# VitorMPCastro/MessyerRaytracer

Measured on AMD Instinct MI355X. Metric: Mrays/s (primary, closest-hit), higher is better.
Workload: dtype f32

## Files before the change

__graft_entry__.py:

```python
import os
import sys

ROOT = os.path.dirname(os.path.abspath(__file__))
if ROOT not in sys.path:
    sys.path.insert(0, ROOT)


def build() -> None:
    from messyerraytracer_amd import build as b
    b.build_lib()
    b.build_host_test()
    b.build_host_cpu_test()
    b.build_host_tlas_test()
    b.build_policy_test()
    b.build_shadow_policy_test()
    b.build_reflection_policy_test()
    b.build_hemisphere_policy_test()
    b.build_bounce_policy_test()
    b.build_instance_math_test()
    b.build_shade_data_test()
    from oracle import pyoracle
    pyoracle.build(force=False)
    if os.path.isdir("/root/reference") and not pyoracle.ref_available():
        pyoracle.build(force=True)
    import messyerraytracer_amd
    from messyerraytracer_amd import capi
    L = capi.load()
    missing = [s for s in capi.SYMBOLS if not hasattr(L, s)]
    if missing:
        raise RuntimeError(f"libmrt_hip.so does not export {missing}")


def smoke() -> None:
    import numpy as np
    from messyerraytracer_amd import capi, synth
    from oracle import pyoracle as po

    ctx = capi.Context(0)
    for verts, (w, h), origin, fwd, fov in (
            (synth.cube(), (16, 12), (0, 0, 3), (0, 0, -1), 60.0),
            (synth.soup(2000, 0.4, 3), (128, 96), (0, 0, -12), (0, 0, 1), 50.0)):
        scene = capi.Scene(verts)
        scene.upload(ctx)
        cam = capi.camera_look(origin, fwd, w, h, fov)
        got = ctx.cast_grid(cam, w, h)
        osc = po.OracleScene(verts)
        rays = po.grid_rays(origin, fwd, w, h, fov)
        want = osc.trace(rays)
        assert (got["prim_id"] == want["prim_id"]).all(), "prim_id mismatch vs oracle"
        hit = want["prim_id"] >= 0
        assert np.array_equal(got["t"][hit], want["t"][hit]), "t mismatch vs oracle"
        assert hit.any() and (~hit).any()
    local, inst = synth.multi_mesh_instances(4, 500, 0.3, 5)
# ... 30 lines not shown
```

messyerraytracer_amd/build.py:

```python
import concurrent.futures
import os
import shutil
import subprocess

HERE = os.path.dirname(os.path.abspath(__file__))
CSRC = os.path.join(HERE, "csrc")
LIB = os.path.join(HERE, "libmrt_hip.so")
OBJ = os.path.join(HERE, "_obj")
HOST_TEST = os.path.join(HERE, "host_mirror_test")
HOST_CPU_TEST = os.path.join(HERE, "host_cpu_test")
HOST_TLAS_TEST = os.path.join(HERE, "host_tlas_test")
POLICY_TEST = os.path.join(HERE, "launch_policy_test")
SHADOW_POLICY_TEST = os.path.join(HERE, "shadow_policy_test")
REFLECTION_POLICY_TEST = os.path.join(HERE, "reflection_policy_test")
HEMISPHERE_POLICY_TEST = os.path.join(HERE, "hemisphere_policy_test")
BOUNCE_POLICY_TEST = os.path.join(HERE, "bounce_policy_test")
INSTANCE_MATH_TEST = os.path.join(HERE, "instance_math_test")
SHADE_DATA_TEST = os.path.join(HERE, "shade_data_test")

SOURCES = ["kernels.hip", "api.hip", "cast.hip", "schedule.hip", "launch_policy.cpp", "group.hip", "device_build.hip", "refit.hip",
           "tlas_device.hip", "surface.hip", "host/shade_data.cpp", "host/scene_prep.cpp", "host/bvh_builder.cpp", "host/two_level_prep.cpp"]
HEADERS = ["mrt_internal.h", "instance_math.h", "mrt_context.h", "launch_policy.h", "packet_kernel.h", "packet_asm_kernel.h", "packet_rows_kernel.h", "packet_quad_kernel.h", "two_level_kernel.h", "lane_persistent_kernel.h", "source_common.h", "shadow_kernel.h", "reflection_kernel.h", "hemisphere_kernel.h", "bounce_kernel.h", "surface_kernel.h", "shade_data.h", "lane_walk.inc", "two_level_walk.inc", "persistent_walk.inc", "../../include/mrt_hip.h", "host/gpu_ray_caster.hpp", "host/ray_dispatcher.hpp",
           "host/host_types.hpp", "host/cpu_backend.hpp", "host/ray_tracer_server.hpp", "host/record_policy_test.h"]
FLAGS = ["--offload-arch=gfx950", "-O3", "-std=c++17", "-fPIC", "-ffp-contract=off", "-Wall",
         "-Wno-unused-result", "-Xarch_host", "-mfma"]


def _hipcc() -> str:
    for c in (shutil.which("hipcc"), "/opt/rocm/bin/hipcc"):
        if c and os.path.exists(c):
            return c
    raise RuntimeError("hipcc not found: libmrt_hip.so cannot be built")


def _stale(target: str, deps) -> bool:
    if not os.path.exists(target):
        return True
    t = os.path.getmtime(target)
    return any(os.path.exists(d) and os.path.getmtime(d) > t for d in deps)


def build_lib(force: bool = False, verbose: bool = False) -> str:
    srcs = [os.path.join(CSRC, s) for s in SOURCES]
    deps = srcs + [os.path.join(CSRC, h) for h in HEADERS] + [os.path.abspath(__file__)]
    if force or _stale(LIB, deps):
        extra = ["-DMRT_WITH_QUAD"] if os.environ.get("MRT_WITH_QUAD") == "1" else []
        extra += os.environ.get("MRT_EXTRA_DEFINES", "").split()
        os.makedirs(OBJ, exist_ok=True)
        objs = [os.path.join(OBJ, s.replace("/", "_") + ".o") for s in SOURCES]

        def compile_one(job):
            src, obj = job
            cmd = [_hipcc()] + FLAGS + extra + ["-c", src, "-o", obj]
            r = subprocess.run(cmd, capture_output=True, text=True, cwd=CSRC)
            if r.returncode != 0:
# ... 92 lines not shown


def build_bounce_policy_test(force: bool = False) -> str:
    srcs = [os.path.join(CSRC, "host", "bounce_policy_test.cpp"), os.path.join(CSRC, "launch_policy.cpp")]
    deps = srcs + [os.path.join(CSRC, h) for h in HEADERS]
    if force or _stale(BOUNCE_POLICY_TEST, deps):
        cmd = [_hipcc(), "-O2", "-std=c++17", "-Wall"] + srcs + ["-o", BOUNCE_POLICY_TEST]
        r = subprocess.run(cmd, capture_output=True, text=True, cwd=CSRC)
        if r.returncode != 0:
            raise RuntimeError("bounce policy test build failed:\n" + r.stdout + r.stderr)
    return BOUNCE_POLICY_TEST


def build_instance_math_test(force: bool = False) -> str:
    src = os.path.join(CSRC, "host", "instance_math_test.cpp")
    deps = [src, os.path.join(CSRC, "instance_math.h")]
    if force or _stale(INSTANCE_MATH_TEST, deps):
        cmd = [_hipcc(), "-x", "c++", "-O2", "-std=c++17", "-ffp-contract=off", "-Wall", src, "-o", INSTANCE_MATH_TEST]
        r = subprocess.run(cmd, capture_output=True, text=True, cwd=CSRC)
        if r.returncode != 0:
            raise RuntimeError("instance math test build failed:\n" + r.stdout + r.stderr)
    return INSTANCE_MATH_TEST


def build_shade_data_test(force: bool = False) -> str:
    srcs = [os.path.join(CSRC, "host", "shade_data_test.cpp"), os.path.join(CSRC, "host", "shade_data.cpp")]
    deps = srcs + [os.path.join(CSRC, "shade_data.h"), os.path.join(CSRC, "../../include/mrt_hip.h")]
    if force or _stale(SHADE_DATA_TEST, deps):
        cmd = [_hipcc(), "-x", "c++", "-O2", "-std=c++17", "-ffp-contract=off", "-Wall"] + srcs + ["-o", SHADE_DATA_TEST]
        r = subprocess.run(cmd, capture_output=True, text=True, cwd=CSRC)
        if r.returncode != 0:
            raise RuntimeError("shade data test build failed:\n" + r.stdout + r.stderr)
    return SHADE_DATA_TEST


if __name__ == "__main__":
    print(build_lib(force=True, verbose=True))
    print(build_host_test(force=True))
    print(build_host_cpu_test(force=True))
    print(build_host_tlas_test(force=True))
    print(build_policy_test(force=True))
    print(build_shadow_policy_test(force=True))
    print(build_reflection_policy_test(force=True))
    print(build_hemisphere_policy_test(force=True))
    print(build_bounce_policy_test(force=True))
    print(build_instance_math_test(force=True))
    print(build_shade_data_test(force=True))
```

messyerraytracer_amd/csrc/kernels.hip:

```cpp
#include <hip/hip_runtime.h>
#include <cfloat>
#include <cstdarg>
#include <cstdio>
#include <cstdlib>
#include <type_traits>
#include "mrt_internal.h"
#include "shade_data.h"

namespace mrt {

#define MRT_WG 256
#define MRT_WAVE 64

__device__ __forceinline__ float fma_(float a, float b, float c) { return __builtin_fmaf(a, b, c); }
__device__ __forceinline__ float dot3(float ax, float ay, float az, float bx, float by, float bz)
{
	return fma_(ax, bx, fma_(ay, by, az * bz));
}
__device__ __forceinline__ float safe_inv(float d)
{
	const float eps = 1e-9f;
	const float big = 1.0f / eps;
	return __builtin_fabsf(d) > eps ? 1.0f / d : (d >= 0.0f ? big : -big);
}

struct RayRegs {
	float ox, oy, oz, dx, dy, dz, t_min, t_max;
};

__device__ __forceinline__ bool skip_launch(const TraceParams &p)
{
	return p.skip_flag != nullptr && *p.skip_flag == p.skip_when;
}

__device__ __forceinline__ bool lane_ray_index_g(const TraceParams &p, uint64_t g, uint64_t &ray_idx, uint32_t &px, uint32_t &py);
__device__ __forceinline__ bool lane_ray_index(const TraceParams &p, uint32_t block, uint64_t &ray_idx, uint32_t &px, uint32_t &py)
{
	return lane_ray_index_g(p, (uint64_t)block * MRT_WG + threadIdx.x, ray_idx, px, py);
}
__device__ __forceinline__ bool xcd_strips(const TraceParams &p, uint64_t tile, uint32_t tiles_x, uint32_t tiles_y, uint32_t &tx, uint32_t &ty)
{
	const uint32_t tg = p.tile_group ? p.tile_group : 1u;
	uint32_t m = (tiles_x + 128u) >> 8;
	if (m == 0u) m = 1u;
	const uint32_t S = tiles_x / (8u * m);
	if (S == 0u || S * 8u * m != tiles_x || S % tg != 0u) return false;
	const uint64_t wg = tile / tg;
	const uint32_t k = (uint32_t)wg & 7u;
	const uint64_t j = (wg >> 3) * tg + tile % tg;
	const uint64_t per_strip = (uint64_t)S * tiles_y;
	const uint32_t sl = (uint32_t)(j / per_strip), r = (uint32_t)(j % per_strip);
	ty = r / S;
	tx = (sl * 8u + k) * S + r % S;
	return true;
}

__device__ __forceinline__ bool lane_ray_index_g(const TraceParams &p, uint64_t g, uint64_t &ray_idx, uint32_t &px, uint32_t &py)
{
	uint32_t lane_map = p.lane_map, grid_w = p.grid_w, rows = p.rows, tiles_x = p.tiles_x;
	if (lane_map == MAP_AUTO) {
		const uint32_t w = p.auto_grid[0];
		lane_map = w ? MAP_TILE8X8 : MAP_LINEAR;
		grid_w = w; rows = p.auto_grid[1]; tiles_x = p.auto_grid[2];
	}
	if (lane_map == MAP_TILE8X8) {
		uint64_t tile = g >> 6;
		const uint32_t l = (uint32_t)g & 63u;
		uint32_t tx, ty;
		const uint32_t k = p.tile_w_log2;
		const uint32_t tiles_y = (rows + (64u >> k) - 1u) >> (6u - k);
		uint32_t quarter = 4u;
		uint32_t sixteenth = 16u;
		if (p.quarter_all == 2u) { sixteenth = (uint32_t)tile & 15u; tile >>= 4; if (l >= 4u || tile >= (uint64_t)tiles_x * tiles_y) return false; }
		else if (p.quarter_all) { quarter = (uint32_t)tile & 3u; tile >>= 2; if (l >= 16u || tile >= (uint64_t)tiles_x * tiles_y) return false; }
		else if (p.tile_sched != nullptr && ((uint64_t)tiles_x * tiles_y + p.tile_unit - 1u) / p.tile_unit == p.n_units) {
			const uint64_t slot = tile / p.tile_unit;
			if (slot >= (p.sched_hdr ? p.sched_hdr[2] : p.n_units)) return false;
			const uint32_t e = p.tile_sched[slot], what = e >> 28, id = e & 0x0FFFFFFFu;
			if (what == 0u) tile = (uint64_t)id * p.tile_unit + tile % p.tile_unit;
			else {
				if (tile % p.tile_unit != 0u) return false;
				tile = id;
				if (what >= 2u) { quarter = what - 2u; if (l >= 16u) return false; }
			}
		}
		if (p.tile_order == 1u && (tiles_x & 15u) == 0u && (tiles_y & 15u) == 0u) {
			const uint32_t st = (uint32_t)(tile >> 8), in = (uint32_t)tile & 255u;
			uint32_t mx = in & 0x55u, my = (in >> 1) & 0x55u;
			mx = (mx | (mx >> 1)) & 0x33u; mx = (mx | (mx >> 2)) & 0x0Fu;
			my = (my | (my >> 1)) & 0x33u; my = (my | (my >> 2)) & 0x0Fu;
			const uint32_t stx = st % (tiles_x >> 4), sty = st / (tiles_x >> 4);
			tx = (stx << 4) + mx; ty = (sty << 4) + my;
		} else if (p.tile_order == 2u && (tiles_x & 31u) == 0u && (tiles_y & 31u) == 0u) {
			const uint32_t st = (uint32_t)(tile >> 10), in = (uint32_t)tile & 1023u;
			uint32_t mx = in & 0x155u, my = (in >> 1) & 0x155u;
			mx = (mx | (mx >> 1)) & 0x133u; mx = (mx | (mx >> 2)) & 0x10Fu; mx = (mx | (mx >> 4)) & 0x1Fu;
			my = (my | (my >> 1)) & 0x133u; my = (my | (my >> 2)) & 0x10Fu; my = (my | (my >> 4)) & 0x1Fu;
			const uint32_t stx = st % (tiles_x >> 5), sty = st / (tiles_x >> 5);
			tx = (stx << 5) + mx; ty = (sty << 5) + my;
		} else if (p.tile_order == 3u && xcd_strips(p, tile, tiles_x, tiles_y, tx, ty)) {
		} else { tx = (uint32_t)(tile % tiles_x); ty = (uint32_t)(tile / tiles_x); }
		if (sixteenth < 16u) {
			px = (tx << 3) + ((sixteenth & 3u) << 1) + (l & 1u);
			py = (ty << 3) + ((sixteenth >> 2) << 1) + (l >> 1);
		} else if (quarter < 4u) {
			px = (tx << 3) + ((quarter & 1u) << 2) + (l & 3u);
			py = (ty << 3) + ((quarter >> 1) << 2) + (l >> 2);
		} else {
			px = (tx << k) + (l & ((1u << k) - 1u));
			py = (ty << (6u - k)) + (l >> k);
		}
		if (px >= grid_w || py >= rows) return false;
		ray_idx = (uint64_t)py * grid_w + px;
		return true;
	}
	if (p.sparse_lanes) { const uint32_t l = (uint32_t)g & 63u; if (l >= p.sparse_lanes) return false; g = (g >> 6) * p.sparse_lanes + l; }
	if (g >= p.count) return false;
	ray_idx = p.perm ? (uint64_t)p.perm[g] : g;
	if (p.in_fmt == IN_GRID) { px = (uint32_t)(ray_idx % p.grid_w); py = (uint32_t)(ray_idx / p.grid_w); }
	return true;
}

__device__ __forceinline__ bool tile_cost_word(const TraceParams &p, uint64_t g_first, uint32_t *&park, uint32_t *&sum, uint32_t &what)
{
	if (p.tile_cost == nullptr) return false;
	uint32_t rows = p.rows, tiles_x = p.tiles_x;
	if (p.lane_map == MAP_AUTO) { if (p.auto_grid[0] == 0u) return false; rows = p.auto_grid[1]; tiles_x = p.auto_grid[2]; }
	else if (p.lane_map != MAP_TILE8X8) return false;
	const uint32_t k = p.tile_w_log2, tiles_y = (rows + (64u >> k) - 1u) >> (6u - k);
	if (((uint64_t)tiles_x * tiles_y + p.tile_unit - 1u) / p.tile_unit != p.n_units) return false;
	const uint64_t slot = (g_first >> 6) / p.tile_unit;
	what = 0u;
	if (p.tile_sched == nullptr) { if (slot >= p.n_units) return false; park = sum = p.tile_cost + slot; return true; }
	if (slot >= (p.sched_hdr ? p.sched_hdr[2] : p.n_units)) return false;
	const uint32_t e = p.tile_sched[slot], id = e & 0x0FFFFFFFu;
	what = e >> 28;
	if (what == 0u) { park = sum = p.tile_cost + id; return true; }
	park = p.tile_cost + p.n_units + slot;
	sum = p.tile_cost + id / p.tile_unit;
	return true;
}
__device__ __forceinline__ void note_tile_start(const TraceParams &p, uint64_t g_first)
{
	uint32_t *park, *sum, what;
	if (tile_cost_word(p, g_first, park, sum, what)) *park = (uint32_t)__builtin_amdgcn_s_memtime();
}
__device__ __forceinline__ void note_tile_cost(const TraceParams &p, uint64_t g_first)
{
	uint32_t *park, *sum, what;
	if (!tile_cost_word(p, g_first, park, sum, what)) return;
	uint32_t d = (uint32_t)__builtin_amdgcn_s_memtime() - *park;
	if (park == sum) { *sum = d ? d : 1u; return; }
	if (what == 1u) d = d - (d >> 2);
	else d = p.tile_unit == 2u ? (d >> 1) + (d >> 3) + (d >> 4) : d - (d >> 3);
	atomicAdd(sum, d ? d : 1u);
}

__device__ __forceinline__ void grid_ray(const TraceParams &p, uint32_t px, uint32_t py, RayRegs &r)
{
	const mrt_camera &c = p.cam;
	float dx, dy, dz;
	r.ox = c.origin[0]; r.oy = c.origin[1]; r.oz = c.origin[2];
	if (c.kind == MRT_CAMERA_DEBUG_GRID) {
		const float u = (2.0f * ((float)px + 0.5f) / (float)p.grid_w - 1.0f) * c.half_w;
		const float v = (2.0f * ((float)(py + p.y0) + 0.5f) / (float)p.grid_h - 1.0f) * c.half_h;
		dx = c.fwd[0] + c.right[0] * u + c.up[0] * v;
		dy = c.fwd[1] + c.right[1] * u + c.up[1] * v;
		dz = c.fwd[2] + c.right[2] * u + c.up[2] * v;
	} else {
		const float u = (2.0f * ((float)px + c.jitter_x) * c.inv_w) - 1.0f;
		const float v = 1.0f - (2.0f * ((float)(py + p.y0) + c.jitter_y) * c.inv_h);
		if (c.kind == MRT_CAMERA_PERSPECTIVE) {
			const float vx = u * c.half_w, vy = v * c.half_h;
			dx = c.right[0] * vx + c.up[0] * vy + c.fwd[0] * -1.0f;
			dy = c.right[1] * vx + c.up[1] * vy + c.fwd[1] * -1.0f;
			dz = c.right[2] * vx + c.up[2] * vy + c.fwd[2] * -1.0f;
		} else {
			const float sv = v * c.half_h, su = u * c.half_w;
			r.ox = (c.origin[0] + c.up[0] * sv) + c.right[0] * su;
			r.oy = (c.origin[1] + c.up[1] * sv) + c.right[1] * su;
			r.oz = (c.origin[2] + c.up[2] * sv) + c.right[2] * su;
			r.dx = -c.fwd[0]; r.dy = -c.fwd[1]; r.dz = -c.fwd[2];
			r.t_min = c.t_min; r.t_max = c.t_max;
			return;
		}
	}
	const float l2 = dx * dx + dy * dy + dz * dz;
	if (l2 == 0.0f) { dx = dy = dz = 0.0f; }
	else { const float l = __builtin_sqrtf(l2); dx /= l; dy /= l; dz /= l; }
	r.dx = dx; r.dy = dy; r.dz = dz;
	r.t_min = c.t_min; r.t_max = c.t_max;
}

__device__ __forceinline__ void load_ray(const TraceParams &p, uint64_t idx, uint32_t px, uint32_t py, RayRegs &r)
{
	if (p.in_fmt == IN_GRID) { grid_ray(p, px, py, r); return; }
	float ox, oy, oz, dx, dy, dz, t0, t1;
	if (p.in_fmt == IN_HOST60) {
		const float *h = reinterpret_cast<const float *>(p.rays) + idx * 15u;
		ox = h[0]; oy = h[1]; oz = h[2]; dx = h[3]; dy = h[4]; dz = h[5];
		t0 = h[12]; t1 = h[13];
	} else {
		const float4 *q = reinterpret_cast<const float4 *>(p.rays) + idx * 2u;
		const float4 a = q[0], b = q[1];
		ox = a.x; oy = a.y; oz = a.z; t1 = a.w;
		dx = b.x; dy = b.y; dz = b.z; t0 = b.w;
	}
	r.ox = ox; r.oy = oy; r.oz = oz; r.dx = dx; r.dy = dy; r.dz = dz; r.t_min = t0; r.t_max = t1;
}

__device__ __forceinline__ void store_hit(const TraceParams &p, uint64_t idx, const RayRegs &r,
		float t, int32_t prim, float u, float v, float nx, float ny, float nz, uint32_t layers, uint32_t slot)
{
	if (p.out_fmt == OUT_BOOL8) { reinterpret_cast<uint8_t *>(p.hits)[idx] = prim >= 0 ? 1 : 0; return; }
	if (p.out_fmt == OUT_TOKEN4) { reinterpret_cast<uint32_t *>(p.hits)[idx] = prim >= 0 ? slot : 0xFFFFFFFFu; return; }
	if (p.out_fmt == OUT_HOST44) {
		float *h = reinterpret_cast<float *>(p.hits) + idx * 11u;
		uint32_t *hu = reinterpret_cast<uint32_t *>(h);
		if (prim >= 0) {
			h[0] = t;
			h[1] = r.ox + r.dx * t; h[2] = r.oy + r.dy * t; h[3] = r.oz + r.dz * t;
			h[4] = nx; h[5] = ny; h[6] = nz; h[7] = u; h[8] = v;
			hu[9] = (uint32_t)prim; hu[10] = layers;
		} else {
			h[0] = FLT_MAX; h[1] = h[2] = h[3] = 0.0f; h[4] = h[5] = h[6] = 0.0f; h[7] = h[8] = 0.0f;
			hu[9] = 0xFFFFFFFFu; hu[10] = 0u;
		}
		return;
	}
	float4 *q = reinterpret_cast<float4 *>(p.hits) + idx * 2u;
	float4 a, b;
	a.x = t; a.y = __int_as_float(prim); a.z = u; a.w = v;
	b.x = nx; b.y = ny; b.z = nz; b.w = __uint_as_float(layers);
	q[0] = a; q[1] = b;
}

__device__ __forceinline__ void finish_ray(const TraceParams &p, uint64_t ray_idx, const RayRegs &r,
		float best_t, float best_u, float best_v, uint32_t best_slot)
{
	int32_t prim = -1; float nx = 0.0f, ny = 0.0f, nz = 0.0f; uint32_t layers = 0u;
	if (best_slot != 0xFFFFFFFFu) {
		if (p.out_fmt == OUT_BOOL8 || p.out_fmt == OUT_TOKEN4) prim = 0;
		else {
			prim = (int32_t)p.tri_hot[best_slot].id;
			layers = p.tri_hot[best_slot].layers;
			const float4 nn = reinterpret_cast<const float4 *>(p.tri_cold)[best_slot];
			nx = nn.x; ny = nn.y; nz = nn.z;
		}
	}
	store_hit(p, ray_idx, r, best_t, prim, best_u, best_v, nx, ny, nz, layers, best_slot);
}

__device__ __forceinline__ void finish_two_level_ray(const TraceParams &p, uint64_t ray_idx, const RayRegs &r,
		float best_t, float best_u, float best_v, uint32_t best_slot, uint32_t best_id, uint32_t best_inst)
{
	int32_t prim = -1; float nx = 0.0f, ny = 0.0f, nz = 0.0f; uint32_t layers = 0u;
	if (p.out_fmt == OUT_TOKEN8) {
		reinterpret_cast<uint2 *>(p.hits)[ray_idx] = make_uint2(best_slot, best_slot != 0xFFFFFFFFu ? best_inst : 0u);
		return;
	}
	if (best_slot != 0xFFFFFFFFu) {
		prim = (int32_t)best_id;
		if (p.out_fmt != OUT_BOOL8) {
			const float4 *row = reinterpret_cast<const float4 *>(p.instances) + (size_t)best_inst * 8u;
			const float4 b0 = row[3], b1 = row[4], b2 = row[5];
			const float4 no = reinterpret_cast<const float4 *>(p.tri_cold)[best_slot];
			nx = fma_(b0.x, no.x, fma_(b0.y, no.y, b0.z * no.z));
// ... 631 lines not shown
```

messyerraytracer_amd/csrc/packet_rows_kernel.h:

```cpp
#pragma once

#define RA_LMINX "s20"
#define RA_LMINY "s21"
#define RA_LMINZ "s22"
#define RA_LREF "s23"
#define RA_LMAXX "s24"
#define RA_LMAXY "s25"
#define RA_LMAXZ "s26"
#define RA_RREF "s27"
#define RA_RMINX "s28"
#define RA_RMINY "s29"
#define RA_RMINZ "s30"
#define RA_RMAXX "s32"
#define RA_RMAXY "s33"
#define RA_RMAXZ "s34"
#define RA_MASK "s[60:61]"
#define RA_MASKLO "s60"
#define RA_MASKHI "s61"
#define RA_V0X "s20"
#define RA_V0Y "s21"
#define RA_V0Z "s22"
#define RA_ID "s23"
#define RA_E1X "s24"
#define RA_E1Y "s25"
// ... 646 lines not shown
	if (__ballot(!inside) != 0ull || !planes_ok) return c;
	const float n1 = __builtin_fabsf(n[0]) + __builtin_fabsf(n[1]) + __builtin_fabsf(n[2]);
	const float o1 = __builtin_fabsf(ox) + __builtin_fabsf(oy) + __builtin_fabsf(oz);
	const float err = 8.0f * 5.9604645e-8f * n1 * (scene_abs_max + o1);
	const float cc = (n[0] * ox + n[1] * oy + n[2] * oz) - err;
	if (__ballot(!__builtin_isfinite(cc)) != 0ull) return c;
	const uint32_t d = lane & 15u, axis = d & 3u;
	const bool is_max = (d >> 2 & 1u) != 0u;
	const float na = axis == 0u ? n[0] : (axis == 1u ? n[1] : n[2]);
	c.w = (axis < 3u && ((na >= 0.0f) == is_max)) ? na : 0.0f;
	c.cc = (d == 7u || d == 15u) ? cc : -__builtin_inff();
	return c;
}

__device__ __forceinline__ void rows_init(PacketRegs &s, const RayRegs &r, bool takes_part, uint32_t sp)
{
	s.ox = r.ox; s.oy = r.oy; s.oz = r.oz; s.dx = r.dx; s.dy = r.dy; s.dz = r.dz; s.tmin = r.t_min;
	s.ix = safe_inv(r.dx); s.iy = safe_inv(r.dy); s.iz = safe_inv(r.dz);
	s.nrx = -(r.ox * s.ix); s.nry = -(r.oy * s.iy); s.nrz = -(r.oz * s.iz);
	s.bt = r.t_max; s.bu = 0.0f; s.bv = 0.0f; s.bs = 0xFFFFFFFFu; s.bi = 0xFFFFFFFFu;
	s.lim = (!takes_part || r.t_min >= r.t_max) ? -FLT_MAX : r.t_max;
	s.sp = sp; s.cur = 0u; s.mask = 0ull;
}

__device__ __forceinline__ int rows_octant(const RayRegs &r, bool part, unsigned long long &part_mask)
{
	part_mask = __ballot(part);
	const unsigned long long sx = __ballot(part && safe_inv(r.dx) < 0.0f), sy = __ballot(part && safe_inv(r.dy) < 0.0f),
			sz = __ballot(part && safe_inv(r.dz) < 0.0f);
	const bool uniform = (sx == 0ull || sx == part_mask) && (sy == 0ull || sy == part_mask) && (sz == 0ull || sz == part_mask);
	return uniform ? ((sx ? 1 : 0) | (sy ? 2 : 0) | (sz ? 4 : 0)) : 8;
}

#ifndef MRT_ROWS_WPE
#define MRT_ROWS_WPE 8
#endif
template <bool ANY_HIT, bool COUNT, int PACKETS, int WG, bool CULL = false>
__global__ __launch_bounds__(WG) __attribute__((amdgpu_waves_per_eu(MRT_ROWS_WPE, 8))) void trace_packet_rows_kernel(const TraceParams p)
{
	__shared__ __attribute__((aligned(16))) uint32_t wave_stack[WG / MRT_WAVE][PACKETS][(MRT_PACKET_STACK + 1) * 4];
	if (skip_launch(p)) return;
	uint32_t block = blockIdx.x;
	if (p.xcd_swizzle) {
		const uint32_t per = gridDim.x >> 3;
		if (block < (per << 3)) block = (block & 7u) * per + (block >> 3);
	}
	const uint32_t wave = threadIdx.x / MRT_WAVE, lane = threadIdx.x & (MRT_WAVE - 1);
	const uint32_t wave_s = __builtin_amdgcn_readfirstlane(wave), block_s = block;
	const uint64_t g_a = (((uint64_t)block * (WG / MRT_WAVE) + wave) * PACKETS) * MRT_WAVE + lane, g_b = g_a + MRT_WAVE;
	uint64_t idx = 0; uint32_t px = 0, py = 0;
	const bool valid_a = lane_ray_index_g(p, g_a, idx, px, py);
	RayRegs ra = {0.0f, 0.0f, 0.0f, 0.0f, 0.0f, 0.0f, 1.0f, 0.0f}, rb = ra;
	if (valid_a) load_ray(p, idx, px, py, ra);
	bool valid_b = false;
	if (PACKETS == 2) {
		valid_b = lane_ray_index_g(p, g_b, idx, px, py);
		if (valid_b) load_ray(p, idx, px, py, rb);
	}
	if (__ballot(valid_a || valid_b) == 0ull) return;

	const float4 *rows = reinterpret_cast<const float4 *>(p.row_array);
	uint32_t *stack_a = wave_stack[wave][0], *stack_b = wave_stack[wave][PACKETS - 1];
	*(volatile uint32_t *)&stack_a[0] = kSentinel;
	if (PACKETS == 2) *(volatile uint32_t *)&stack_b[0] = kSentinel;
	PacketRegs A, B;
	rows_init(A, ra, valid_a, (uint32_t)(uintptr_t)(__attribute__((address_space(3))) uint32_t *)(stack_a + 4));
	rows_init(B, rb, valid_b, (uint32_t)(uintptr_t)(__attribute__((address_space(3))) uint32_t *)(stack_b + 4));

	unsigned long long part_a = 0ull, part_b = 0ull;
	const int oct_a = rows_octant(ra, valid_a, part_a);
	const int oct_b = PACKETS == 2 ? rows_octant(rb, valid_b, part_b) : 8;
	uint32_t cnt_n = 0u, cnt_t = 0u;
	uint32_t cnt_w = 0u;
	uint32_t sp_wide = 0u, sp_one = 0u;
	if (p.tile_cost != nullptr && lane == 0u) note_tile_start(p, g_a);
	if (COUNT) *(volatile unsigned long long *)&stack_a[2] = __builtin_amdgcn_s_memtime();
	bool done_a = part_a == 0ull, done_b = part_b == 0ull;
	if (PACKETS == 2 && !done_a && !done_b && oct_a == oct_b && oct_a != 8) {
		*(volatile uint32_t *)&stack_a[4] = kSentinel;
		A.sp += 16u;
		A.mask = part_a; B.mask = part_b;
		if (CULL) {
			const CullRegs cull = cull_setup(ra, rb, valid_a, valid_b, part_a, part_b, p.scene_abs_max, lane);
#define MRT_RWC(O) case O: rows_walk_cull<O, ANY_HIT, COUNT>(rows, p.query_mask, A, B, cull, cnt_n, cnt_t, sp_wide); break;
			switch (oct_a) { MRT_RWC(0) MRT_RWC(1) MRT_RWC(2) MRT_RWC(3) MRT_RWC(4) MRT_RWC(5) MRT_RWC(6) MRT_RWC(7) }
#undef MRT_RWC
		} else {
#define MRT_RW2(O) case O: rows_walk_wide<O, ANY_HIT, COUNT>(rows, p.query_mask, A, B, cnt_n, cnt_t, sp_wide); break;
		switch (oct_a) { MRT_RW2(0) MRT_RW2(1) MRT_RW2(2) MRT_RW2(3) MRT_RW2(4) MRT_RW2(5) MRT_RW2(6) MRT_RW2(7) }
#undef MRT_RW2
		}
		done_a = done_b = true;
	}
#define MRT_RW1(O, S) case O: rows_walk_one<O, ANY_HIT, COUNT>(rows, p.query_mask, S, cnt_n, cnt_t, cnt_w, sp_one); break;
	if (!done_a && oct_a != 8) { switch (oct_a) { MRT_RW1(0, A) MRT_RW1(1, A) MRT_RW1(2, A) MRT_RW1(3, A) MRT_RW1(4, A) MRT_RW1(5, A) MRT_RW1(6, A) MRT_RW1(7, A) } done_a = true; }
	if (PACKETS == 2 && !done_b && oct_b != 8) { switch (oct_b) { MRT_RW1(0, B) MRT_RW1(1, B) MRT_RW1(2, B) MRT_RW1(3, B) MRT_RW1(4, B) MRT_RW1(5, B) MRT_RW1(6, B) MRT_RW1(7, B) } done_b = true; }
#undef MRT_RW1
	uint32_t slot_a = A.bs == 0xFFFFFFFFu ? 0xFFFFFFFFu : A.bs - p.n_nodes, slot_b = B.bs == 0xFFFFFFFFu ? 0xFFFFFFFFu : B.bs - p.n_nodes;
	if (!done_a) {
		uint32_t nn = 0, nt = 0, nd = 0;
		A.bt = ra.t_max;
		packet_traverse<8, ANY_HIT, COUNT>(p, ra, stack_a, A.bt, A.bu, A.bv, slot_a, nn, nt, nd, 0u, 0u, nullptr, !valid_a);
		if (COUNT) { cnt_n += __builtin_amdgcn_readfirstlane(nn); cnt_t += __builtin_amdgcn_readfirstlane(nt); }
	}
	if (PACKETS == 2 && !done_b) {
		uint32_t nn = 0, nt = 0, nd = 0;
		B.bt = rb.t_max;
		packet_traverse<8, ANY_HIT, COUNT>(p, rb, stack_b, B.bt, B.bu, B.bv, slot_b, nn, nt, nd, 0u, 0u, nullptr, !valid_b);
		if (COUNT) { cnt_n += __builtin_amdgcn_readfirstlane(nn); cnt_t += __builtin_amdgcn_readfirstlane(nt); }
	}

	{
		const uint32_t lane2 = __builtin_amdgcn_mbcnt_hi(~0u, __builtin_amdgcn_mbcnt_lo(~0u, 0u));
		const uint64_t h_a = (((uint64_t)block_s * (WG / MRT_WAVE) + wave_s) * PACKETS) * MRT_WAVE + lane2;
		uint64_t idx2 = 0; uint32_t px2 = 0, py2 = 0;
		if (lane_ray_index_g(p, h_a, idx2, px2, py2)) finish_ray(p, idx2, ra, A.bt, A.bu, A.bv, slot_a);
		if (PACKETS == 2 && lane_ray_index_g(p, h_a + MRT_WAVE, idx2, px2, py2)) finish_ray(p, idx2, rb, B.bt, B.bu, B.bv, slot_b);
		if (p.tile_cost != nullptr && lane2 == 0u) note_tile_cost(p, h_a);
	}
	const unsigned long long t_start = COUNT ? *(volatile unsigned long long *)&stack_a[2] : 0ull;
	if (COUNT && lane == 0u && (p.count_mode != 2u || (blockIdx.x & 15u) == 0u)) {
		atomicAdd(&p.counters[kCntFetchWaitCycles], (unsigned long long)cnt_w);
		atomicAdd(&p.counters[kCntWaveCycles], __builtin_amdgcn_s_memtime() - t_start);
		atomicAdd(&p.counters[kCntWaves], 1ull);
	}
	if (COUNT && p.count_mode != 2u) {
		const uint32_t base = (uint32_t)(uintptr_t)(__attribute__((address_space(3))) uint32_t *)stack_a;
		const uint32_t e_wide = sp_wide > base ? (sp_wide - base) / 32u : 0u, e_one = sp_one > base ? ((sp_one - base) % 1040u) / 16u : 0u;
		atomicMax(&p.counters[kCntMaxStack], (unsigned long long)(e_wide > e_one ? e_wide : e_one));
	}
	if (COUNT && p.count_mode != 2u) {
		if (valid_a) packet_count(p, cnt_n, cnt_t, 0u, slot_a != 0xFFFFFFFFu, part_a | part_b);
		if (PACKETS == 2 && valid_b) { atomicAdd(&p.counters[kCntRays], 1ull); if (slot_b != 0xFFFFFFFFu) atomicAdd(&p.counters[kCntHits], 1ull); }
	}
}
```

Before: 8628.

## Compute wave tile once per wave and stream ray I/O with nontemporal access

Moves the lane-to-pixel mapping into a shared header that computes each wave's tile once and derives the second packet's tile incrementally, instead of redoing the full per-lane mapping for each load and store. The rows kernel also gains a finish path that reads the hit normal and prim id from the row data using the winning slot, and, for single-wave workgroups, uses nontemporal loads and stores for ray input and hit output. The aim is to cut integer index arithmetic and cache pollution from streaming ray buffers. The cost is more code-path complexity and some risk of divergence from the old mapping in edge cases such as schedules and quarter tiles.

```diff
diff --git a/__graft_entry__.py b/__graft_entry__.py
--- a/__graft_entry__.py
+++ b/__graft_entry__.py
@@ -19,6 +19,7 @@
     b.build_bounce_policy_test()
     b.build_instance_math_test()
     b.build_shade_data_test()
+    b.build_lane_map_test()
     from oracle import pyoracle
     pyoracle.build(force=False)
     if os.path.isdir("/root/reference") and not pyoracle.ref_available():
diff --git a/messyerraytracer_amd/build.py b/messyerraytracer_amd/build.py
--- a/messyerraytracer_amd/build.py
+++ b/messyerraytracer_amd/build.py
@@ -17,10 +17,11 @@
 BOUNCE_POLICY_TEST = os.path.join(HERE, "bounce_policy_test")
 INSTANCE_MATH_TEST = os.path.join(HERE, "instance_math_test")
 SHADE_DATA_TEST = os.path.join(HERE, "shade_data_test")
+LANE_MAP_TEST = os.path.join(HERE, "lane_map_test")
 
 SOURCES = ["kernels.hip", "api.hip", "cast.hip", "schedule.hip", "launch_policy.cpp", "group.hip", "device_build.hip", "refit.hip",
            "tlas_device.hip", "surface.hip", "host/shade_data.cpp", "host/scene_prep.cpp", "host/bvh_builder.cpp", "host/two_level_prep.cpp"]
-HEADERS = ["mrt_internal.h", "instance_math.h", "mrt_context.h", "launch_policy.h", "packet_kernel.h", "packet_asm_kernel.h", "packet_rows_kernel.h", "packet_quad_kernel.h", "two_level_kernel.h", "lane_persistent_kernel.h", "source_common.h", "shadow_kernel.h", "reflection_kernel.h", "hemisphere_kernel.h", "bounce_kernel.h", "surface_kernel.h", "shade_data.h", "lane_walk.inc", "two_level_walk.inc", "persistent_walk.inc", "../../include/mrt_hip.h", "host/gpu_ray_caster.hpp", "host/ray_dispatcher.hpp",
+HEADERS = ["mrt_internal.h", "instance_math.h", "lane_map.h", "mrt_context.h", "launch_policy.h", "packet_kernel.h", "packet_asm_kernel.h", "packet_rows_kernel.h", "packet_quad_kernel.h", "two_level_kernel.h", "lane_persistent_kernel.h", "source_common.h", "shadow_kernel.h", "reflection_kernel.h", "hemisphere_kernel.h", "bounce_kernel.h", "surface_kernel.h", "shade_data.h", "lane_walk.inc", "two_level_walk.inc", "persistent_walk.inc", "../../include/mrt_hip.h", "host/gpu_ray_caster.hpp", "host/ray_dispatcher.hpp",
            "host/host_types.hpp", "host/cpu_backend.hpp", "host/ray_tracer_server.hpp", "host/record_policy_test.h"]
 FLAGS = ["--offload-arch=gfx950", "-O3", "-std=c++17", "-fPIC", "-ffp-contract=off", "-Wall",
          "-Wno-unused-result", "-Xarch_host", "-mfma"]
@@ -179,6 +180,19 @@
         if r.returncode != 0:
             raise RuntimeError("shade data test build failed:\n" + r.stdout + r.stderr)
     return SHADE_DATA_TEST
+
+
+def build_lane_map_test(force: bool = False, sanitize: bool = False) -> str:
+    src = os.path.join(CSRC, "host", "lane_map_test.cpp")
+    exe = LANE_MAP_TEST + ("_san" if sanitize else "")
+    deps = [src, os.path.join(CSRC, "lane_map.h")]
+    if force or _stale(exe, deps):
+        flags = ["-O1", "-g", "-fno-omit-frame-pointer", "-fsanitize=address,undefined", "-fno-sanitize-recover=undefined"] if sanitize else ["-O2"]
+        cmd = [_hipcc(), "-x", "c++", "-std=c++17", "-Wall"] + flags + [src, "-o", exe]
+        r = subprocess.run(cmd, capture_output=True, text=True, cwd=CSRC)
+        if r.returncode != 0:
+            raise RuntimeError("lane map test build failed:\n" + r.stdout + r.stderr)
+    return exe
 
 
 if __name__ == "__main__":
@@ -193,3 +207,4 @@
     print(build_bounce_policy_test(force=True))
     print(build_instance_math_test(force=True))
     print(build_shade_data_test(force=True))
+    print(build_lane_map_test(force=True))
diff --git a/messyerraytracer_amd/csrc/kernels.hip b/messyerraytracer_amd/csrc/kernels.hip
--- a/messyerraytracer_amd/csrc/kernels.hip
+++ b/messyerraytracer_amd/csrc/kernels.hip
@@ -6,6 +6,7 @@
 #include <type_traits>
 #include "mrt_internal.h"
 #include "shade_data.h"
+#include "lane_map.h"
 
 namespace mrt {
 
@@ -38,87 +39,39 @@
 {
 	return lane_ray_index_g(p, (uint64_t)block * MRT_WG + threadIdx.x, ray_idx, px, py);
 }
-__device__ __forceinline__ bool xcd_strips(const TraceParams &p, uint64_t tile, uint32_t tiles_x, uint32_t tiles_y, uint32_t &tx, uint32_t &ty)
-{
-	const uint32_t tg = p.tile_group ? p.tile_group : 1u;
-	uint32_t m = (tiles_x + 128u) >> 8;
-	if (m == 0u) m = 1u;
-	const uint32_t S = tiles_x / (8u * m);
-	if (S == 0u || S * 8u * m != tiles_x || S % tg != 0u) return false;
-	const uint64_t wg = tile / tg;
-	const uint32_t k = (uint32_t)wg & 7u;
-	const uint64_t j = (wg >> 3) * tg + tile % tg;
-	const uint64_t per_strip = (uint64_t)S * tiles_y;
-	const uint32_t sl = (uint32_t)(j / per_strip), r = (uint32_t)(j % per_strip);
-	ty = r / S;
-	tx = (sl * 8u + k) * S + r % S;
-	return true;
-}
-
-__device__ __forceinline__ bool lane_ray_index_g(const TraceParams &p, uint64_t g, uint64_t &ray_idx, uint32_t &px, uint32_t &py)
-{
-	uint32_t lane_map = p.lane_map, grid_w = p.grid_w, rows = p.rows, tiles_x = p.tiles_x;
+
+__device__ __forceinline__ bool tile_grid(const TraceParams &p, TileGrid &g)
+{
+	uint32_t lane_map = p.lane_map;
+	g.grid_w = p.grid_w; g.rows = p.rows; g.tiles_x = p.tiles_x;
 	if (lane_map == MAP_AUTO) {
 		const uint32_t w = p.auto_grid[0];
 		lane_map = w ? MAP_TILE8X8 : MAP_LINEAR;
-		grid_w = w; rows = p.auto_grid[1]; tiles_x = p.auto_grid[2];
-	}
-	if (lane_map == MAP_TILE8X8) {
-		uint64_t tile = g >> 6;
-		const uint32_t l = (uint32_t)g & 63u;
-		uint32_t tx, ty;
-		const uint32_t k = p.tile_w_log2;
-		const uint32_t tiles_y = (rows + (64u >> k) - 1u) >> (6u - k);
-		uint32_t quarter = 4u;
-		uint32_t sixteenth = 16u;
-		if (p.quarter_all == 2u) { sixteenth = (uint32_t)tile & 15u; tile >>= 4; if (l >= 4u || tile >= (uint64_t)tiles_x * tiles_y) return false; }
-		else if (p.quarter_all) { quarter = (uint32_t)tile & 3u; tile >>= 2; if (l >= 16u || tile >= (uint64_t)tiles_x * tiles_y) return false; }
-		else if (p.tile_sched != nullptr && ((uint64_t)tiles_x * tiles_y + p.tile_unit - 1u) / p.tile_unit == p.n_units) {
-			const uint64_t slot = tile / p.tile_unit;
-			if (slot >= (p.sched_hdr ? p.sched_hdr[2] : p.n_units)) return false;
-			const uint32_t e = p.tile_sched[slot], what = e >> 28, id = e & 0x0FFFFFFFu;
-			if (what == 0u) tile = (uint64_t)id * p.tile_unit + tile % p.tile_unit;
-			else {
-				if (tile % p.tile_unit != 0u) return false;
-				tile = id;
-				if (what >= 2u) { quarter = what - 2u; if (l >= 16u) return false; }
-			}
-		}
-		if (p.tile_order == 1u && (tiles_x & 15u) == 0u && (tiles_y & 15u) == 0u) {
-			const uint32_t st = (uint32_t)(tile >> 8), in = (uint32_t)tile & 255u;
-			uint32_t mx = in & 0x55u, my = (in >> 1) & 0x55u;
-			mx = (mx | (mx >> 1)) & 0x33u; mx = (mx | (mx >> 2)) & 0x0Fu;
-			my = (my | (my >> 1)) & 0x33u; my = (my | (my >> 2)) & 0x0Fu;
-			const uint32_t stx = st % (tiles_x >> 4), sty = st / (tiles_x >> 4);
-			tx = (stx << 4) + mx; ty = (sty << 4) + my;
-		} else if (p.tile_order == 2u && (tiles_x & 31u) == 0u && (tiles_y & 31u) == 0u) {
-			const uint32_t st = (uint32_t)(tile >> 10), in = (uint32_t)tile & 1023u;
-			uint32_t mx = in & 0x155u, my = (in >> 1) & 0x155u;
-			mx = (mx | (mx >> 1)) & 0x133u; mx = (mx | (mx >> 2)) & 0x10Fu; mx = (mx | (mx >> 4)) & 0x1Fu;
-			my = (my | (my >> 1)) & 0x133u; my = (my | (my >> 2)) & 0x10Fu; my = (my | (my >> 4)) & 0x1Fu;
-			const uint32_t stx = st % (tiles_x >> 5), sty = st / (tiles_x >> 5);
-			tx = (stx << 5) + mx; ty = (sty << 5) + my;
-		} else if (p.tile_order == 3u && xcd_strips(p, tile, tiles_x, tiles_y, tx, ty)) {
-		} else { tx = (uint32_t)(tile % tiles_x); ty = (uint32_t)(tile / tiles_x); }
-		if (sixteenth < 16u) {
-			px = (tx << 3) + ((sixteenth & 3u) << 1) + (l & 1u);
-			py = (ty << 3) + ((sixteenth >> 2) << 1) + (l >> 1);
-		} else if (quarter < 4u) {
-			px = (tx << 3) + ((quarter & 1u) << 2) + (l & 3u);
-			py = (ty << 3) + ((quarter >> 1) << 2) + (l >> 2);
-		} else {
-			px = (tx << k) + (l & ((1u << k) - 1u));
-			py = (ty << (6u - k)) + (l >> k);
-		}
-		if (px >= grid_w || py >= rows) return false;
-		ray_idx = (uint64_t)py * grid_w + px;
-		return true;
-	}
-	if (p.sparse_lanes) { const uint32_t l = (uint32_t)g & 63u; if (l >= p.sparse_lanes) return false; g = (g >> 6) * p.sparse_lanes + l; }
-	if (g >= p.count) return false;
-	ray_idx = p.perm ? (uint64_t)p.perm[g] : g;
+		g.grid_w = w; g.rows = p.auto_grid[1]; g.tiles_x = p.auto_grid[2];
+	}
+	g.k = p.tile_w_log2; g.tiles_y = tile_rows_of(g.rows, g.k);
+	g.order = p.tile_order; g.group = p.tile_group; g.quarter_all = p.quarter_all;
+	g.sched = nullptr; g.unit = 1u; g.sched_slots = 0u;
+	if (lane_map != MAP_TILE8X8) return false;
+	if (!p.quarter_all && p.tile_sched != nullptr && sched_matches((uint64_t)g.tiles_x * g.tiles_y, p.tile_unit, p.n_units)) {
+		g.sched = p.tile_sched; g.unit = p.tile_unit; g.sched_slots = p.sched_hdr ? p.sched_hdr[2] : p.n_units;
+	}
+	return true;
+}
+__device__ __forceinline__ bool linear_ray(const TraceParams &p, uint64_t group, uint32_t l, uint64_t &ray_idx, uint32_t &px, uint32_t &py)
+{
+	uint64_t e = 0;
+	if (!linear_lane(group, l, p.sparse_lanes, p.count, e)) return false;
+	ray_idx = p.perm ? (uint64_t)p.perm[e] : e;
 	if (p.in_fmt == IN_GRID) { px = (uint32_t)(ray_idx % p.grid_w); py = (uint32_t)(ray_idx / p.grid_w); }
 	return true;
+}
+
+__device__ __forceinline__ bool lane_ray_index_g(const TraceParams &p, uint64_t g, uint64_t &ray_idx, uint32_t &px, uint32_t &py)
+{
+	TileGrid tg;
+	if (tile_grid(p, tg)) return tile_lane(tg, wave_tile(tg, g >> 6), (uint32_t)g & 63u, ray_idx, px, py);
+	return linear_ray(p, g >> 6, (uint32_t)g & 63u, ray_idx, px, py);
 }
 
 __device__ __forceinline__ bool tile_cost_word(const TraceParams &p, uint64_t g_first, uint32_t *&park, uint32_t *&sum, uint32_t &what)
@@ -128,8 +81,9 @@
 	if (p.lane_map == MAP_AUTO) { if (p.auto_grid[0] == 0u) return false; rows = p.auto_grid[1]; tiles_x = p.auto_grid[2]; }
 	else if (p.lane_map != MAP_TILE8X8) return false;
 	const uint32_t k = p.tile_w_log2, tiles_y = (rows + (64u >> k) - 1u) >> (6u - k);
-	if (((uint64_t)tiles_x * tiles_y + p.tile_unit - 1u) / p.tile_unit != p.n_units) return false;
-	const uint64_t slot = (g_first >> 6) / p.tile_unit;
+	if (!sched_matches((uint64_t)tiles_x * tiles_y, p.tile_unit, p.n_units)) return false;
+	const uint64_t group = g_first >> 6;
+	const uint64_t slot = p.tile_unit == 1u ? group : (p.tile_unit == 2u ? group >> 1 : group / p.tile_unit);
 	what = 0u;
 	if (p.tile_sched == nullptr) { if (slot >= p.n_units) return false; park = sum = p.tile_cost + slot; return true; }
 	if (slot >= (p.sched_hdr ? p.sched_hdr[2] : p.n_units)) return false;
@@ -192,6 +146,19 @@
 	r.t_min = c.t_min; r.t_max = c.t_max;
 }
 
+typedef float mrt_v4f __attribute__((ext_vector_type(4)));
+__device__ __forceinline__ float4 stream_load4(const float4 *q)
+{
+	const mrt_v4f v = __builtin_nontemporal_load(reinterpret_cast<const mrt_v4f *>(q));
+	return make_float4(v.x, v.y, v.z, v.w);
+}
+__device__ __forceinline__ void stream_store4(float4 *q, const float4 &a)
+{
+	const mrt_v4f v = {a.x, a.y, a.z, a.w};
+	__builtin_nontemporal_store(v, reinterpret_cast<mrt_v4f *>(q));
+}
+
+template <bool STREAM = false>
 __device__ __forceinline__ void load_ray(const TraceParams &p, uint64_t idx, uint32_t px, uint32_t py, RayRegs &r)
 {
 	if (p.in_fmt == IN_GRID) { grid_ray(p, px, py, r); return; }
@@ -202,13 +169,14 @@
 		t0 = h[12]; t1 = h[13];
 	} else {
 		const float4 *q = reinterpret_cast<const float4 *>(p.rays) + idx * 2u;
-		const float4 a = q[0], b = q[1];
+		const float4 a = STREAM ? stream_load4(q) : q[0], b = STREAM ? stream_load4(q + 1) : q[1];
 		ox = a.x; oy = a.y; oz = a.z; t1 = a.w;
 		dx = b.x; dy = b.y; dz = b.z; t0 = b.w;
 	}
 	r.ox = ox; r.oy = oy; r.oz = oz; r.dx = dx; r.dy = dy; r.dz = dz; r.t_min = t0; r.t_max = t1;
 }
 
+template <bool STREAM = false>
 __device__ __forceinline__ void store_hit(const TraceParams &p, uint64_t idx, const RayRegs &r,
 		float t, int32_t prim, float u, float v, float nx, float ny, float nz, uint32_t layers, uint32_t slot)
 {
@@ -232,7 +200,8 @@
 	float4 a, b;
 	a.x = t; a.y = __int_as_float(prim); a.z = u; a.w = v;
 	b.x = nx; b.y = ny; b.z = nz; b.w = __uint_as_float(layers);
-	q[0] = a; q[1] = b;
+	if (STREAM) { stream_store4(q, a); stream_store4(q + 1, b); }
+	else { q[0] = a; q[1] = b; }
 }
 
 __device__ __forceinline__ void finish_ray(const TraceParams &p, uint64_t ray_idx, const RayRegs &r,
diff --git a/messyerraytracer_amd/csrc/lane_map.h b/messyerraytracer_amd/csrc/lane_map.h
--- /dev/null
+++ b/messyerraytracer_amd/csrc/lane_map.h
@@ -0,0 +1,165 @@
+#pragma once
+#include <cstdint>
+
+#if defined(__HIPCC__) || defined(__HIP__)
+#define MRT_LM_HD __host__ __device__ __forceinline__
+#else
+#define MRT_LM_HD inline
+#endif
+
+namespace mrt {
+
+struct TileGrid {
+	uint32_t grid_w, rows;
+	uint32_t tiles_x, tiles_y;
+	uint32_t k;
+	uint32_t order;
+	uint32_t group;
+	uint32_t quarter_all;
+	const uint32_t *sched;
+	uint32_t unit, sched_slots;
+};
+
+constexpr uint32_t kPieceTile = 20u, kPieceTile16 = 21u, kPieceNone = 0xFFu;
+constexpr uint32_t kNextAnew = 0u, kNextSame = 1u, kNextRight = 2u, kNextRowMajor = 3u, kNextNone = 4u;
+struct WaveTile {
+	uint32_t tx, ty;
+	uint32_t code;
+};
+
+MRT_LM_HD uint32_t tile_rows_of(uint32_t rows, uint32_t k) { return (rows + (64u >> k) - 1u) >> (6u - k); }
+
+MRT_LM_HD bool sched_matches(uint64_t total, uint32_t unit, uint32_t n_units)
+{
+	if (n_units == 0u) return total == 0u;
+	return (uint64_t)(n_units - 1u) * unit < total && total <= (uint64_t)n_units * unit;
+}
+
+template <class T>
+MRT_LM_HD bool strip_tile(const TileGrid &g, T tile, uint32_t &tx, uint32_t &ty)
+{
+	const uint32_t tg = g.group ? g.group : 1u;
+	uint32_t m = (g.tiles_x + 128u) >> 8;
+	if (m == 0u) m = 1u;
+	const uint32_t S = g.tiles_x / (8u * m);
+	if (S == 0u || S * 8u * m != g.tiles_x || S % tg != 0u) return false;
+	const T wg = tile / tg;
+	const uint32_t x = (uint32_t)wg & 7u;
+	const T j = (wg >> 3) * tg + (tile - wg * tg);
+	const T per_strip = (T)S * g.tiles_y;
+	const T q = j / per_strip;
+	const uint32_t sl = (uint32_t)q, r = (uint32_t)(j - q * per_strip);
+	ty = r / S;
+	tx = (sl * 8u + x) * S + r % S;
+	return true;
+}
+
+template <class T>
+MRT_LM_HD WaveTile wave_tile_t(const TileGrid &g, T group)
+{
+	WaveTile w; w.tx = 0u; w.ty = 0u; w.code = kPieceNone;
+	const T total = (T)g.tiles_x * g.tiles_y;
+	T tile = group;
+	uint32_t piece = kPieceTile, next = kNextAnew;
+	bool plus1 = false;
+	if (g.quarter_all == 2u) {
+		piece = (uint32_t)tile & 15u; tile >>= 4;
+		if (tile >= total) return w;
+		if (piece < 15u) next = kNextSame;
+	} else if (g.quarter_all) {
+		piece = 16u + ((uint32_t)tile & 3u); tile >>= 2;
+		if (tile >= total) return w;
+		if (piece < 19u) next = kNextSame;
+	} else if (g.sched != nullptr) {
+		const T slot = g.unit == 1u ? tile : (g.unit == 2u ? tile >> 1 : tile / g.unit);
+		const uint32_t rem = (uint32_t)(tile - slot * g.unit);
+		if (slot >= g.sched_slots) return w;
+		const uint32_t e = g.sched[slot], what = e >> 28, id = e & 0x0FFFFFFFu;
+		if (what == 0u) { tile = (T)id * g.unit + rem; plus1 = rem + 1u < g.unit; }
+		else {
+			if (rem != 0u) return w;
+			tile = id;
+			if (what >= 2u) piece = what - 2u < 4u ? 16u + (what - 2u) : kPieceTile16;
+			if (g.unit > 1u) next = kNextNone;
+		}
+	} else plus1 = true;
+	const bool even = ((uint32_t)tile & 1u) == 0u;
+	if (g.order == 1u && (g.tiles_x & 15u) == 0u && (g.tiles_y & 15u) == 0u) {
+		const uint32_t st = (uint32_t)(tile >> 8), in = (uint32_t)tile & 255u;
+		uint32_t mx = in & 0x55u, my = (in >> 1) & 0x55u;
+		mx = (mx | (mx >> 1)) & 0x33u; mx = (mx | (mx >> 2)) & 0x0Fu;
+		my = (my | (my >> 1)) & 0x33u; my = (my | (my >> 2)) & 0x0Fu;
+		const uint32_t sx = g.tiles_x >> 4, sty = st / sx;
+		w.tx = ((st - sty * sx) << 4) + mx; w.ty = (sty << 4) + my;
+		if (plus1 && even) next = kNextRight;
+	} else if (g.order == 2u && (g.tiles_x & 31u) == 0u && (g.tiles_y & 31u) == 0u) {
+		const uint32_t st = (uint32_t)(tile >> 10), in = (uint32_t)tile & 1023u;
+		uint32_t mx = in & 0x155u, my = (in >> 1) & 0x155u;
+		mx = (mx | (mx >> 1)) & 0x133u; mx = (mx | (mx >> 2)) & 0x10Fu; mx = (mx | (mx >> 4)) & 0x1Fu;
+		my = (my | (my >> 1)) & 0x133u; my = (my | (my >> 2)) & 0x10Fu; my = (my | (my >> 4)) & 0x1Fu;
+		const uint32_t sx = g.tiles_x >> 5, sty = st / sx;
+		w.tx = ((st - sty * sx) << 5) + mx; w.ty = (sty << 5) + my;
+		if (plus1 && even) next = kNextRight;
+	} else if (g.order == 3u && strip_tile<T>(g, tile, w.tx, w.ty)) {
+		if (plus1 && even && g.group != 0u && (g.group & 1u) == 0u) next = kNextRight;
+	} else {
+		const T y = tile / g.tiles_x;
+		w.tx = (uint32_t)(tile - y * g.tiles_x); w.ty = (uint32_t)y;
+		if (plus1) next = kNextRowMajor;
+	}
+	w.code = piece | next << 8;
+	return w;
+}
+
+MRT_LM_HD WaveTile wave_tile(const TileGrid &g, uint64_t group)
+{
+	const bool narrow = (group >> 32) == 0u && (((uint64_t)g.tiles_x * g.tiles_y) >> 32) == 0u && (g.sched == nullptr || g.unit <= 16u);
+	return narrow ? wave_tile_t<uint32_t>(g, (uint32_t)group) : wave_tile_t<uint64_t>(g, group);
+}
+
+MRT_LM_HD WaveTile wave_tile_next(const TileGrid &g, const WaveTile &a, uint64_t group)
+{
+	WaveTile b = a;
+	const uint32_t piece = a.code & 0xFFu, next = piece == kPieceNone ? kNextAnew : a.code >> 8;
+	b.code = piece | kNextAnew << 8;
+	if (next == kNextSame) { b.code += 1u; return b; }
+	if (next == kNextNone) { b.code = kPieceNone; return b; }
+	if (next == kNextRight) { b.tx = a.tx + 1u; return b; }
+	if (next == kNextRowMajor) {
+		b.tx = a.tx + 1u;
+		if (b.tx == g.tiles_x) { b.tx = 0u; b.ty = a.ty + 1u; }
+		return b;
+	}
+	return wave_tile(g, group + 1u);
+}
+
+MRT_LM_HD bool tile_lane(const TileGrid &g, const WaveTile &w, uint32_t l, uint64_t &ray_idx, uint32_t &px, uint32_t &py)
+{
+	const uint32_t piece = w.code & 0xFFu;
+	if (piece == kPieceNone) return false;
+	if (piece < 16u) {
+		if (l >= 4u) return false;
+		px = (w.tx << 3) + ((piece & 3u) << 1) + (l & 1u);
+		py = (w.ty << 3) + ((piece >> 2) << 1) + (l >> 1);
+	} else if (piece < kPieceTile) {
+		if (l >= 16u) return false;
+		px = (w.tx << 3) + ((piece & 1u) << 2) + (l & 3u);
+		py = (w.ty << 3) + (((piece >> 1) & 1u) << 2) + (l >> 2);
+	} else {
+		if (piece == kPieceTile16 && l >= 16u) return false;
+		px = (w.tx << g.k) + (l & ((1u << g.k) - 1u));
+		py = (w.ty << (6u - g.k)) + (l >> g.k);
+	}
+	if (px >= g.grid_w || py >= g.rows) return false;
+	ray_idx = (uint64_t)py * g.grid_w + px;
+	return true;
+}
+
+MRT_LM_HD bool linear_lane(uint64_t group, uint32_t l, uint32_t sparse_lanes, uint64_t count, uint64_t &entry)
+{
+	if (sparse_lanes) { if (l >= sparse_lanes) return false; entry = group * sparse_lanes + l; }
+	else entry = (group << 6) + l;
+	return entry < count;
+}
+
+}
diff --git a/messyerraytracer_amd/csrc/packet_rows_kernel.h b/messyerraytracer_amd/csrc/packet_rows_kernel.h
--- a/messyerraytracer_amd/csrc/packet_rows_kernel.h
+++ b/messyerraytracer_amd/csrc/packet_rows_kernel.h
@@ -702,6 +702,30 @@
 	return uniform ? ((sx ? 1 : 0) | (sy ? 2 : 0) | (sz ? 4 : 0)) : 8;
 }
 
+__device__ __forceinline__ void rows_hit_of_slot(const float4 *rows, uint32_t n_nodes, uint32_t slot, PacketRegs &s)
+{
+	s.bs = 0xFFFFFFFFu;
+	if (slot != 0xFFFFFFFFu) { s.bs = slot + n_nodes; s.bi = __float_as_uint(rows[(size_t)s.bs * 4u].w); }
+}
+
+template <bool STREAM>
+__device__ __forceinline__ void finish_row_ray(const TraceParams &p, const float4 *rows, uint64_t ray_idx, const RayRegs &r,
+		float best_t, float best_u, float best_v, uint32_t best_row, uint32_t best_id, uint32_t best_slot)
+{
+	int32_t prim = -1; float nx = 0.0f, ny = 0.0f, nz = 0.0f; uint32_t layers = 0u;
+	if (best_row != 0xFFFFFFFFu) {
+		if (p.out_fmt == OUT_BOOL8 || p.out_fmt == OUT_TOKEN4) prim = 0;
+		else {
+			const float4 *row = rows + (size_t)best_row * 4u;
+			prim = (int32_t)best_id;
+			layers = __float_as_uint(reinterpret_cast<const float *>(row)[7]);
+			const float4 nn = row[3];
+			nx = nn.x; ny = nn.y; nz = nn.z;
+		}
+	}
+	store_hit<STREAM>(p, ray_idx, r, best_t, prim, best_u, best_v, nx, ny, nz, layers, best_slot);
+}
+
 #ifndef MRT_ROWS_WPE
 #define MRT_ROWS_WPE 8
 #endif
@@ -710,6 +734,7 @@
 {
 	__shared__ __attribute__((aligned(16))) uint32_t wave_stack[WG / MRT_WAVE][PACKETS][(MRT_PACKET_STACK + 1) * 4];
 	if (skip_launch(p)) return;
+	constexpr bool STREAM = WG == MRT_WAVE;
 	uint32_t block = blockIdx.x;
 	if (p.xcd_swizzle) {
 		const uint32_t per = gridDim.x >> 3;
@@ -717,15 +742,25 @@
 	}
 	const uint32_t wave = threadIdx.x / MRT_WAVE, lane = threadIdx.x & (MRT_WAVE - 1);
 	const uint32_t wave_s = __builtin_amdgcn_readfirstlane(wave), block_s = block;
-	const uint64_t g_a = (((uint64_t)block * (WG / MRT_WAVE) + wave) * PACKETS) * MRT_WAVE + lane, g_b = g_a + MRT_WAVE;
+	const uint64_t group_a = ((uint64_t)block_s * (WG / MRT_WAVE) + wave_s) * PACKETS;
+	TileGrid tg;
+	const bool tiled = tile_grid(p, tg);
+	WaveTile ta = {0u, 0u, kPieceNone}, tb = ta;
+	if (tiled) {
+		ta = wave_tile(tg, group_a);
+		if (PACKETS == 2) tb = wave_tile_next(tg, ta, group_a);
+	}
+	const uint32_t tile_ax = __builtin_amdgcn_readfirstlane(ta.tx), tile_ay = __builtin_amdgcn_readfirstlane(ta.ty);
+	const uint32_t tile_bx = __builtin_amdgcn_readfirstlane(tb.tx), tile_by = __builtin_amdgcn_readfirstlane(tb.ty);
+	const uint32_t tile_code = __builtin_amdgcn_readfirstlane((ta.code & 0xFFu) | (tb.code & 0xFFu) << 8 | (tiled ? 1u << 16 : 0u));
 	uint64_t idx = 0; uint32_t px = 0, py = 0;
-	const bool valid_a = lane_ray_index_g(p, g_a, idx, px, py);
+	const bool valid_a = tiled ? tile_lane(tg, ta, lane, idx, px, py) : linear_ray(p, group_a, lane, idx, px, py);
 	RayRegs ra = {0.0f, 0.0f, 0.0f, 0.0f, 0.0f, 0.0f, 1.0f, 0.0f}, rb = ra;
-	if (valid_a) load_ray(p, idx, px, py, ra);
+	if (valid_a) load_ray<STREAM>(p, idx, px, py, ra);
 	bool valid_b = false;
 	if (PACKETS == 2) {
-		valid_b = lane_ray_index_g(p, g_b, idx, px, py);
-		if (valid_b) load_ray(p, idx, px, py, rb);
+		valid_b = tiled ? tile_lane(tg, tb, lane, idx, px, py) : linear_ray(p, group_a + 1u, lane, idx, px, py);
+		if (valid_b) load_ray<STREAM>(p, idx, px, py, rb);
 	}
 	if (__ballot(valid_a || valid_b) == 0ull) return;
 
@@ -743,7 +778,7 @@
 	uint32_t cnt_n = 0u, cnt_t = 0u;
 	uint32_t cnt_w = 0u;
 	uint32_t sp_wide = 0u, sp_one = 0u;
-	if (p.tile_cost != nullptr && lane == 0u) note_tile_start(p, g_a);
+	if (p.tile_cost != nullptr && lane == 0u) note_tile_start(p, group_a << 6);
 	if (COUNT) *(volatile unsigned long long *)&stack_a[2] = __builtin_amdgcn_s_memtime();
 	bool done_a = part_a == 0ull, done_b = part_b == 0ull;
 	if (PACKETS == 2 && !done_a && !done_b && oct_a == oct_b && oct_a != 8) {
@@ -772,21 +807,29 @@
 		A.bt = ra.t_max;
 		packet_traverse<8, ANY_HIT, COUNT>(p, ra, stack_a, A.bt, A.bu, A.bv, slot_a, nn, nt, nd, 0u, 0u, nullptr, !valid_a);
 		if (COUNT) { cnt_n += __builtin_amdgcn_readfirstlane(nn); cnt_t += __builtin_amdgcn_readfirstlane(nt); }
+		rows_hit_of_slot(rows, p.n_nodes, slot_a, A);
 	}
 	if (PACKETS == 2 && !done_b) {
 		uint32_t nn = 0, nt = 0, nd = 0;
 		B.bt = rb.t_max;
 		packet_traverse<8, ANY_HIT, COUNT>(p, rb, stack_b, B.bt, B.bu, B.bv, slot_b, nn, nt, nd, 0u, 0u, nullptr, !valid_b);
 		if (COUNT) { cnt_n += __builtin_amdgcn_readfirstlane(nn); cnt_t += __builtin_amdgcn_readfirstlane(nt); }
+		rows_hit_of_slot(rows, p.n_nodes, slot_b, B);
 	}
 
 	{
 		const uint32_t lane2 = __builtin_amdgcn_mbcnt_hi(~0u, __builtin_amdgcn_mbcnt_lo(~0u, 0u));
-		const uint64_t h_a = (((uint64_t)block_s * (WG / MRT_WAVE) + wave_s) * PACKETS) * MRT_WAVE + lane2;
+		const uint64_t h_a = ((uint64_t)block_s * (WG / MRT_WAVE) + wave_s) * PACKETS;
+		const bool tiled2 = (tile_code >> 16 & 1u) != 0u;
+		TileGrid tg2;
+		(void)tile_grid(p, tg2);
+		const WaveTile ua = {tile_ax, tile_ay, tile_code & 0xFFu}, ub = {tile_bx, tile_by, tile_code >> 8 & 0xFFu};
 		uint64_t idx2 = 0; uint32_t px2 = 0, py2 = 0;
-		if (lane_ray_index_g(p, h_a, idx2, px2, py2)) finish_ray(p, idx2, ra, A.bt, A.bu, A.bv, slot_a);
-		if (PACKETS == 2 && lane_ray_index_g(p, h_a + MRT_WAVE, idx2, px2, py2)) finish_ray(p, idx2, rb, B.bt, B.bu, B.bv, slot_b);
-		if (p.tile_cost != nullptr && lane2 == 0u) note_tile_cost(p, h_a);
+		if (tiled2 ? tile_lane(tg2, ua, lane2, idx2, px2, py2) : linear_ray(p, h_a, lane2, idx2, px2, py2))
+			finish_row_ray<STREAM>(p, rows, idx2, ra, A.bt, A.bu, A.bv, A.bs, A.bi, slot_a);
+		if (PACKETS == 2 && (tiled2 ? tile_lane(tg2, ub, lane2, idx2, px2, py2) : linear_ray(p, h_a + 1u, lane2, idx2, px2, py2)))
+			finish_row_ray<STREAM>(p, rows, idx2, rb, B.bt, B.bu, B.bv, B.bs, B.bi, slot_b);
+		if (p.tile_cost != nullptr && lane2 == 0u) note_tile_cost(p, h_a << 6);
 	}
 	const unsigned long long t_start = COUNT ? *(volatile unsigned long long *)&stack_a[2] : 0ull;
 	if (COUNT && lane == 0u && (p.count_mode != 2u || (blockIdx.x & 15u) == 0u)) {
```

After: 9327, median of 6. 1.08x the previous value.
